# SanPen/CSparse3

Measured on AMD Instinct MI355X. Metric: numeric-LU + lsolve/usolve nnz/s on 50k power-grid Jacobian, higher is better.
Workload: dtype f64; 1 GPU; configs[2]: synthetic banded power-grid Jacobian 50000x50000, 501330 nnz, LU refactor + 1-RHS solve per step, one matrix per GPU; n=50000, nnz_a=501330, nnz_l=696852, nnz_u=696852, rhs=1, supernodes=5970, levels=12, max_front=469, ordering=amd(A+A')

## Files before the change

csparse3_amd/csrc/kernels.hip:

```cpp
#include <hip/hip_runtime.h>


#include <stdint.h>

#include <algorithm>
#include <cstdlib>

#include "cs3_device.hpp"
#include "cs3_devfn.hpp"

namespace cs3 {

hipError_t set_withhold_handover(int on)
{
    hipError_t e = hipMemcpyToSymbol(HIP_SYMBOL(g_withhold_handover), &on, sizeof(int));
    return e != hipSuccess ? e : set_withhold_handover_forest(on);
}

typedef double double4_t __attribute__((ext_vector_type(4)));

__device__ __forceinline__ double *il_lane_base(const IlView &il, long long m)
{
    return il.base + (m >> 6) * 64 * il.len + (m & 63);
}
// ... 2123 lines not shown
        us[j] = load_if(L, off, row < kb && jj < bw);
    }
    {
        constexpr int QW = BIG_KT / 4;
        BlockTriangle<KIND, false> ta;
        ta.load(L, r, kb, bw);
        double vi[QW];
#pragma unroll
        for (int u = 0; u < QW; ++u) {
            const int q = wv * QW + u;
            vi[u] = load_if(v0 + (long long) (q < nlive ? q : 0) * bv_size, kb + lane, lane < bw && q < nlive);
        }
        ta.template solve_multi<QW>(vi, bw);
#pragma unroll
        for (int u = 0; u < QW; ++u) y[wv * QW + u][lane] = (lane < bw) ? vi[u] : 0.0;
    }
    __syncthreads();
    if (blockIdx.x == 0 && tid < bw)
        for (int q = 0; q < nlive; ++q)
            X_all[(long long) b * x_stride + (long long) (d.c0 + kb + tid) * nrhs + rhs0 + q] = y[q][tid];
#pragma unroll
    for (int q = 0; q < BIG_KT; ++q) {
        double acc = 0.0;
#pragma unroll
        for (int j = 0; j < 16; ++j) acc += us[j] * y[q][wv * 16 + j];
        part[wv][q][lane] = acc;
    }
    __syncthreads();
    if (tid < 64 && row < kb)
        for (int q = 0; q < nlive; ++q) {
            double *vq = v0 + (long long) q * bv_size;
            vq[row] -= ((part[0][q][tid] + part[1][q][tid]) + part[2][q][tid]) + part[3][q][tid];
        }
}

template <int KIND>
__global__ void __launch_bounds__(256)
k_bwd_big_init(const SolveDesc *__restrict__ sd, int first, const int *__restrict__ st_idx,
               const double *__restrict__ pool_all, const double *__restrict__ X_all, double *__restrict__ bigv_all,
               int nrhs, long long pool_stride, long long x_stride, long long bv_size)
{
    extern __shared__ __attribute__((aligned(16))) double v2[];
    const SolveDesc d = sd[first + blockIdx.z];
    const int b = blockIdx.y / nrhs, rhs = blockIdx.y % nrhs;
    const int r = d.r, w = d.w, nb = r - w;
    const double *pool = pool_all + (long long) b * pool_stride;
    const double *X = X_all + (long long) b * x_stride;
    double *v = bigv_all + ((long long) b * nrhs + rhs) * bv_size + d.bv;
    const int *st = st_idx + d.st;
    const int tid = threadIdx.x;
    for (int j = tid; j < nb; j += 256) v2[j] = X[(long long) st[w + j] * nrhs + rhs];
    __syncthreads();
    const double *L = pool + d.lpan;
    const double *U = pool + d.upan;
    for (int i = blockIdx.x * 256 + tid; i < w; i += gridDim.x * 256) {
        double acc = 0.0;
        for (int j0 = 0; j0 < nb; j0 += 16) {
            double u[16];
#pragma unroll
            for (int j = 0; j < 16; ++j) {
                const int jj = j0 + j;
                const long long off = (KIND == CS3_LU) ? (long long) i * d.u_sk + (long long) jj * d.u_sj
                                                       : (long long) (w + jj) + (long long) i * r;
                u[j] = load_if((KIND == CS3_LU) ? U : L, off, jj < nb);
            }
#pragma unroll
            for (int j = 0; j < 16; ++j) acc += u[j] * v2[j0 + j < nb ? j0 + j : 0];
        }
        v[i] = X[(long long) (d.c0 + i) * nrhs + rhs] - acc;
    }
}

template <int KIND, int CW>
__global__ void __launch_bounds__(256)
k_bwd_big_step(const SolveDesc *__restrict__ sd, int first, int chunk_from_right,
               const double *__restrict__ pool_all, double *__restrict__ X_all, double *__restrict__ bigv_all,
               int nrhs, long long pool_stride, long long x_stride, long long bv_size)
{
    constexpr int SC = CW / 4;
    __shared__ double y[BIG_CW];
    __shared__ double cpl[64];
    __shared__ double part[4][64];
    const SolveDesc d = sd[first + blockIdx.z];
    const int r = d.r, w = d.w;
    const int nchunk = (w + CW - 1) / CW;
    const int c = nchunk - 1 - chunk_from_right;
    if (c < 0) return;
    const int kb = c * CW, bw = min(CW, w - kb);
    const int bwa = min(SOLVE_BW, bw), bwb = bw - bwa;
    const int nsl = (kb + 63) / 64;
    if ((int) blockIdx.x > 0 && (int) blockIdx.x >= nsl) return;
    const int b = blockIdx.y / nrhs, rhs = blockIdx.y % nrhs;
    const double *L = pool_all + (long long) b * pool_stride + d.lpan;
    double *v = bigv_all + ((long long) b * nrhs + rhs) * bv_size + d.bv;
    const int tid = threadIdx.x, lane = tid & 63, wv = tid >> 6;
    const int row = blockIdx.x * 64 + lane;
    double us[SC];
#pragma unroll
    for (int j = 0; j < SC; ++j) {
        const int jj = wv * SC + j;
        const long long off = (KIND == CS3_LU) ? (long long) row + (long long) (kb + jj) * r
                                               : (long long) (kb + jj) + (long long) row * r;
        us[j] = load_if(L, off, row < kb && jj < bw);
    }
    if (wv == 0) {
        if (bwb > 0) {
            BlockTriangle<KIND, false> tb;
            tb.load(L, r, kb + SOLVE_BW, bwb);
            const double vi = tb.solve(load_if(v, kb + SOLVE_BW + lane, lane < bwb), bwb);
            if (lane < bwb) y[SOLVE_BW + lane] = vi;
        }
        __syncthreads();
        __syncthreads();
    } else if (wv == 1) {
        BlockTriangle<KIND, false> ta;
        ta.load(L, r, kb, bwa);
        __syncthreads();
        __syncthreads();
        const double vi = ta.solve(cpl[lane], bwa);
        if (lane < bwa) y[lane] = vi;
    } else if (wv == 2) {
        double tm[SOLVE_BW];
#pragma unroll
        for (int j = 0; j < SOLVE_BW; ++j) {
            const long long i = kb + lane, k = kb + SOLVE_BW + j;
            const long long off = (KIND == CS3_LU) ? i + k * r : k + i * r;
            tm[j] = load_if(L, off, lane < bwa && j < bwb);
        }
        double vi = load_if(v, kb + lane, lane < bwa);
        __syncthreads();
#pragma unroll
        for (int j = 0; j < SOLVE_BW; ++j) vi -= tm[j] * ((j < bwb) ? y[SOLVE_BW + j] : 0.0);
        cpl[lane] = vi;
        __syncthreads();
    } else {
        __syncthreads();
        __syncthreads();
    }
    __syncthreads();
    if (blockIdx.x == 0 && tid < bw)
        X_all[(long long) b * x_stride + (long long) (d.c0 + kb + tid) * nrhs + rhs] = y[tid];
    double acc = 0.0;
#pragma unroll
    for (int j = 0; j < SC; ++j) {
        const int jj = wv * SC + j;
        acc += us[j] * y[jj < bw ? jj : 0];
    }
    part[wv][lane] = acc;
    __syncthreads();
    if (tid < 64 && row < kb)
        v[row] -= ((part[0][tid] + part[1][tid]) + part[2][tid]) + part[3][tid];
}

constexpr int IL_KB = 4;
constexpr int IL_T = 8;
constexpr int IL_TJ = 4;
constexpr int IL_NONE = INT32_MIN;
constexpr int IL_AV = 32;

template <int KIND, class Rule>
__global__ void __launch_bounds__(64)
k_front_il(const FrontDesc *__restrict__ fdesc, int first, const int *__restrict__ pairs,
           const double *__restrict__ ax_all, long long nnz_a, IlView il,
           const double *__restrict__ pool_pm_all, long long pm_stride, int batch, Rule rule, int *status)
{
    const double inv_tol = rule.inv_tol;
    const FrontDesc d = fdesc[first + blockIdx.x];
    const int lane = threadIdx.x;
    const long long m = (long long) blockIdx.y * 64 + lane;
    const bool live = m < batch;
    const long long mm = live ? m : (long long) blockIdx.y * 64;
    double *G = il.base + (long long) blockIdx.y * 64 * il.len + lane;
    const double *P = pool_pm_all + mm * pm_stride;
    const double *ax = ax_all + mm * nnz_a;
    const int r = d.r, w = d.w;
    double *F = G + d.lpan * 64;
#define EL(i, j) F[((long long) (i) + (long long) (j) * r) * 64]

    {
        const int np = d.a_count;
        const int *pr = pairs + 2 * d.a_begin;
        int cur = -1;
        double acc = 0.0;
        int ptg_n = pr[2 * (lane < min(64, np) ? lane : 0)], psr_n = pr[2 * (lane < min(64, np) ? lane : 0) + 1];
        for (int base = 0; base < np; base += 64) {
            const int have = min(64, np - base);
            const int ptg = ptg_n, psr = psr_n;
            if (base + 64 < np) {
                const int have_n = min(64, np - base - 64);
                const int e_n = base + 64 + (lane < have_n ? lane : 0);
                ptg_n = pr[2 * e_n]; psr_n = pr[2 * e_n + 1];
            }
            for (int c = 0; c < have; c += IL_AV) {
                double val[IL_AV];
#pragma unroll
                for (int u = 0; u < IL_AV; ++u) {
                    const int sr = bcast_lane_i(psr, (c + u) & 63);
                    const bool none = sr == IL_NONE;
                    const int sc = none ? 0 : sr;
                    const double *p = (sc >= 0) ? ((sc < il.len) ? (const double *) (G + (long long) sc * 64) : P + sc) : ax + ~sc;
                    const double v = *p;
                    val[u] = none ? 0.0 : v;
                }
#pragma unroll
                for (int u = 0; u < IL_AV; ++u) {
                    if (c + u >= have) break;
                    const int tg = bcast_lane_i(ptg, c + u);
                    if (tg != cur) {
                        if (cur >= 0) F[(long long) cur * 64] = acc;
                        cur = tg; acc = 0.0;
                    }
                    acc += (tg >= 0) ? val[u] : 0.0;
                }
            }
        }
        if (cur >= 0) F[(long long) cur * 64] = acc;
    }

    bool bad = false;
    int bad_col = 0, hits = 0;
    for (int k0 = 0; k0 < w; k0 += IL_KB) {
        const int kb = min(IL_KB, w - k0), ke = k0 + kb;
        double dd[IL_KB][IL_KB], rd[IL_KB];
#pragma unroll
        for (int jj = 0; jj < IL_KB; ++jj)
#pragma unroll
            for (int ii = 0; ii < IL_KB; ++ii) {
                const bool in = ii < kb && jj < kb && (KIND == CS3_LU || ii >= jj);
                const double v = EL(in ? k0 + ii : k0, in ? k0 + jj : k0);
                dd[jj][ii] = in ? v : ((ii == jj) ? 1.0 : 0.0);
            }
#pragma unroll
        for (int kk = 0; kk < IL_KB; ++kk) {
            double piv = dd[kk][kk];
            if constexpr (Rule::on) {
                if (kk < kb) {
                    const bool hit = perturb_pivot(rule, piv);
                    dd[kk][kk] = piv;
                    hits += (int) hit;
                }
            }
            double dg;
            pivot_scale<KIND>(piv, dg, rd[kk]);
            bool rej = (KIND == CS3_LU) ? (!(fabs(piv) > 0.0) || !(fabs(piv) < 1.0e300)) : !(piv > 0.0);
            if (KIND == CS3_CHOLESKY) dd[kk][kk] = (piv > 0.0) ? dg : -1.0;
#pragma unroll
            for (int ii = kk + 1; ii < IL_KB; ++ii) {
                dd[kk][ii] *= rd[kk];
                if (KIND == CS3_LU) rej = rej || (ii < kb && !(fabs(dd[kk][ii]) <= inv_tol));
            }
            if (rej && kk < kb) { bad_col = bad ? min(bad_col, k0 + kk) : k0 + kk; bad = true; }
#pragma unroll
            for (int jj = kk + 1; jj < IL_KB; ++jj)
#pragma unroll
                for (int ii = (KIND == CS3_LU ? kk + 1 : jj); ii < IL_KB; ++ii)
                    dd[jj][ii] -= dd[kk][ii] * ((KIND == CS3_LU) ? dd[jj][kk] : dd[kk][jj]);
        }
#pragma unroll
        for (int jj = 0; jj < IL_KB; ++jj)
#pragma unroll
            for (int ii = 0; ii < IL_KB; ++ii)
                if (ii < kb && jj < kb && (KIND == CS3_LU || ii >= jj)) EL(k0 + ii, k0 + jj) = dd[jj][ii];
        for (int i0 = ke; i0 < r; i0 += IL_T) {
            double t[IL_T][IL_KB];
#pragma unroll
            for (int a = 0; a < IL_T; ++a)
#pragma unroll
                for (int jj = 0; jj < IL_KB; ++jj) {
                    const bool in = i0 + a < r && jj < kb;
                    const double v = EL(in ? i0 + a : i0, in ? k0 + jj : k0);
                    t[a][jj] = in ? v : 0.0;
                }
#pragma unroll
            for (int a = 0; a < IL_T; ++a)
#pragma unroll
                for (int jj = 0; jj < IL_KB; ++jj) {
                    double x = t[a][jj];
#pragma unroll
                    for (int kk = 0; kk < jj; ++kk) x -= t[a][kk] * ((KIND == CS3_LU) ? dd[jj][kk] : dd[kk][jj]);
                    x *= rd[jj];
                    t[a][jj] = x;
                    if (KIND == CS3_LU && jj < kb && i0 + a < r && !(fabs(x) <= inv_tol)) { bad_col = bad ? min(bad_col, k0 + jj) : k0 + jj; bad = true; }
                }
#pragma unroll
            for (int a = 0; a < IL_T; ++a)
#pragma unroll
                for (int jj = 0; jj < IL_KB; ++jj)
                    if (i0 + a < r && jj < kb) EL(i0 + a, k0 + jj) = t[a][jj];
        }
        if (KIND == CS3_LU) {
            for (int j0 = ke; j0 < r; j0 += IL_T) {
                double u[IL_T][IL_KB];
#pragma unroll
                for (int b = 0; b < IL_T; ++b)
#pragma unroll
                    for (int kk = 0; kk < IL_KB; ++kk) {
                        const bool in = j0 + b < r && kk < kb;
                        const double v = EL(in ? k0 + kk : k0, in ? j0 + b : k0);
                        u[b][kk] = in ? v : 0.0;
                    }
#pragma unroll
                for (int b = 0; b < IL_T; ++b)
#pragma unroll
                    for (int kk = 1; kk < IL_KB; ++kk) {
                        double x = u[b][kk];
#pragma unroll
// ... 882 lines not shown
        break;
    }
    });
#undef CS3_FRONT_ARGS
    CS3_LAUNCH_CHECK();
    return hipSuccess;
}

__global__ void __launch_bounds__(256) k_poison_lds(int words)
{
    extern __shared__ __attribute__((aligned(16))) double pz[];
    for (int i = threadIdx.x; i < words; i += 256) pz[i] = __longlong_as_double(0x7ff8dead0000beefll);
    __syncthreads();
    if (pz[(threadIdx.x * 97) % words] == 0.0) pz[0] = 1.0;
}

hipError_t launch_poison_lds(hipStream_t st)
{
    const int bytes = 160 * 1024;
    hipError_t e = hipFuncSetAttribute((const void *) k_poison_lds, hipFuncAttributeMaxDynamicSharedMemorySize, bytes);
    if (e != hipSuccess) return e;
    hipLaunchKernelGGL(k_poison_lds, dim3(1024), dim3(256), bytes, st, bytes / 8);
    CS3_LAUNCH_CHECK();
    return hipSuccess;
}

hipError_t prepare_kernels()
{
    const int big = 160 * 1024;
    hipError_t e;
    using Plain = PivotRule<false>;
    using Perturbed = PivotRule<true>;
    const void *block_fns[] = {(const void *) k_front_block<CS3_LU, Plain, 16>, (const void *) k_front_block<CS3_LU, Perturbed, 16>,
                               (const void *) k_front_block<CS3_CHOLESKY, Plain, 16>,
                               (const void *) k_front_block<CS3_CHOLESKY, Plain, 16, 4>,
                               (const void *) k_front_wg<CS3_LU, Plain, WG_NB>, (const void *) k_front_wg<CS3_LU, Perturbed, WG_NB>,
                               (const void *) k_front_wg<CS3_CHOLESKY, Plain, WG_NB>};
    for (const void *f : block_fns) {
        e = hipFuncSetAttribute(f, hipFuncAttributeMaxDynamicSharedMemorySize, big);
        if (e != hipSuccess) return e;
    }
    const void *gemm_fns[] = {(const void *) k_gemm_fwd<CS3_LU>, (const void *) k_gemm_fwd<CS3_CHOLESKY>,
                              (const void *) k_gemm_bwd<CS3_LU>, (const void *) k_gemm_bwd<CS3_CHOLESKY>,
                              (const void *) k_gemm_bwd_init<CS3_LU>, (const void *) k_gemm_bwd_init<CS3_CHOLESKY>};
    for (const void *f : gemm_fns) {
        e = hipFuncSetAttribute(f, hipFuncAttributeMaxDynamicSharedMemorySize, big);
        if (e != hipSuccess) return e;
    }
    const void *solve_fns[] = {
        (const void *) k_fwd_blk<CS3_LU>, (const void *) k_fwd_blk<CS3_CHOLESKY>,
        (const void *) k_bwd_blk<CS3_LU>, (const void *) k_bwd_blk<CS3_CHOLESKY>,
        (const void *) k_bwd_big_init<CS3_LU>, (const void *) k_bwd_big_init<CS3_CHOLESKY>};
    for (const void *f : solve_fns) {
        e = hipFuncSetAttribute(f, hipFuncAttributeMaxDynamicSharedMemorySize, big);
        if (e != hipSuccess) return e;
    }
    return hipSuccess;
}

hipError_t ForkJoin::init()
{
    for (int i = 0; i < NSIDE; ++i) {
        hipError_t e = hipStreamCreateWithFlags(&side[i], hipStreamNonBlocking);
        if (e != hipSuccess) return e;
    }
    return hipStreamCreateWithFlags(&aux, hipStreamNonBlocking);
}

void ForkJoin::destroy()
{
    for (int i = 0; i < NSIDE; ++i) if (side[i]) { (void) hipStreamDestroy(side[i]); side[i] = nullptr; }
    if (aux) { (void) hipStreamDestroy(aux); aux = nullptr; }
    for (hipEvent_t e : events) (void) hipEventDestroy(e);
    events.clear();
    next = 0;
}

hipError_t ForkJoin::event(hipEvent_t *out)
{
    if (next == events.size()) {
        hipEvent_t e;
        hipError_t rc = hipEventCreateWithFlags(&e, hipEventDisableTiming);
        if (rc != hipSuccess) return rc;
        events.push_back(e);
    }
    *out = events[next++];
    return hipSuccess;
}

static size_t level_edge(const std::vector<LaunchGroup> &groups, size_t g, bool forward)
{
    const int level = groups[forward ? g : g - 1].level;
    if (forward) while (g < groups.size() && groups[g].level == level) ++g;
    else while (g > 0 && groups[g - 1].level == level) --g;
    return g;
}

template <class F>
static auto with_sweep_kind(int kind, bool trans, F &&f)
{
    if (kind == CS3_LU && trans) return f(std::integral_constant<int, CS3_LU_T>{});
    return with_kind(kind, f);
}

template <class Launch>
static hipError_t run_level(const std::vector<LaunchGroup> &groups, size_t g0, size_t g1, hipStream_t st,
                            ForkJoin &fj, bool parallel, Launch launch)
{
    const size_t ng = g1 - g0;
    if (ng <= 1) return ng ? launch(groups[g0], st) : hipSuccess;
    if (!parallel) {
        for (size_t i = g0; i < g1; ++i) { hipError_t e = launch(groups[i], st); if (e != hipSuccess) return e; }
        return hipSuccess;
    }
    hipEvent_t fork;
    hipError_t e = fj.event(&fork);
    if (e != hipSuccess) return e;
    if ((e = hipEventRecord(fork, st)) != hipSuccess) return e;
    if ((e = launch(groups[g1 - 1], st)) != hipSuccess) return e;
    for (size_t i = 0; i + 1 < ng; ++i) {
        hipStream_t s = fj.side[i % ForkJoin::NSIDE];
        if (i < (size_t) ForkJoin::NSIDE) { if ((e = hipStreamWaitEvent(s, fork, 0)) != hipSuccess) return e; }
        if ((e = launch(groups[g0 + i], s)) != hipSuccess) return e;
    }
    for (size_t i = 0; i < std::min(ng - 1, (size_t) ForkJoin::NSIDE); ++i) {
        hipEvent_t j;
        if ((e = fj.event(&j)) != hipSuccess) return e;
        if ((e = hipEventRecord(j, fj.side[i])) != hipSuccess) return e;
        if ((e = hipStreamWaitEvent(st, j, 0)) != hipSuccess) return e;
    }
    return hipSuccess;
}

static std::vector<LaunchGroup> factor_groups(const DeviceFactor &D, const std::vector<LaunchGroup> &groups);

hipError_t launch_factor_levels(const DeviceFactor &D, const SweepCall &call, const std::vector<LaunchGroup> &all_groups,
                                const PivotCtl &pc, hipStream_t st, ForkJoin &fj)
{
    const std::vector<LaunchGroup> groups = factor_groups(D, all_groups);
    fj.rewind();
    for (size_t g0 = 0; g0 < groups.size(); ) {
        const size_t g1 = level_edge(groups, g0, true);
        hipError_t e = run_level(groups, g0, g1, st, fj, true, [&](const LaunchGroup &g, hipStream_t s) {
            return with_kind(D.kind, [&](auto K) { return launch_front_group<K>(D, call, g, pc, s); });
        });
        if (e != hipSuccess) return e;
        g0 = g1;
    }
    return hipSuccess;
}

struct BigSweepPlan {
    bool wide, multi;
    int cw, nchunk, slices;
    unsigned by, by_multi;
};

static BigSweepPlan big_sweep_plan(const DeviceFactor &D, const LaunchGroup &g, int nrhs)
{
    BigSweepPlan pl;
    pl.by = (unsigned) (D.batch * nrhs);
    pl.wide = (long long) D.batch * nrhs < 8;
    pl.multi = nrhs >= BIG_KT;
    pl.by_multi = (unsigned) (D.batch * ((nrhs + BIG_KT - 1) / BIG_KT));
    pl.cw = pl.wide ? BIG_CW : SOLVE_BW;
    pl.nchunk = (g.max_w + pl.cw - 1) / pl.cw;
    pl.slices = std::max(1, (g.max_r + 63) / 64);
    return pl;
}

static hipError_t launch_fwd_big_pre(const DeviceFactor &D, const SweepCall &call, const LaunchGroup &g, double *X, int nrhs, hipStream_t st)
{
    const BigSweepPlan pl = big_sweep_plan(D, g, nrhs);
    hipLaunchKernelGGL(k_fwd_big_gather, dim3(1, pl.by, g.count), dim3(256), 0, st, call.sd, g.first, D.fasm_src,
                       D.fasm_tgt, D.flong_src, D.cv, X, D.bigv, nrhs, D.cv_size * (long long) nrhs, D.n * (long long) nrhs, D.bv_size);
    CS3_LAUNCH_CHECK();
    return hipSuccess;
}

template <int KIND>
static hipError_t launch_fwd_big_chunk(const DeviceFactor &D, const SweepCall &call, const LaunchGroup &g, double *X, int nrhs, int c,
                                       hipStream_t st)
{
    const BigSweepPlan pl = big_sweep_plan(D, g, nrhs);
    const long long xs = D.n * (long long) nrhs, cvs = D.cv_size * (long long) nrhs;
    if (pl.wide)
        hipLaunchKernelGGL((k_fwd_big_step<KIND, BIG_CW>), dim3(pl.slices, pl.by, g.count), dim3(256), 0, st, call.sd,
                           g.first, c * pl.cw, D.pool_pm, D.cv, X, D.bigv, nrhs, D.pm_stride, cvs, xs, D.bv_size);
    else if (pl.multi)
        hipLaunchKernelGGL((k_fwd_big_step_multi<KIND>), dim3(pl.slices, pl.by_multi, g.count), dim3(256), 0, st, call.sd,
                           g.first, c * pl.cw, D.pool_pm, D.cv, X, D.bigv, nrhs, D.pm_stride, cvs, xs, D.bv_size);
    else
        hipLaunchKernelGGL((k_fwd_big_step<KIND, SOLVE_BW>), dim3(pl.slices, pl.by, g.count), dim3(256), 0, st, call.sd,
                           g.first, c * pl.cw, D.pool_pm, D.cv, X, D.bigv, nrhs, D.pm_stride, cvs, xs, D.bv_size);
    CS3_LAUNCH_CHECK();
    return hipSuccess;
}

template <int KIND>
static hipError_t launch_bwd_big_pre(const DeviceFactor &D, const SweepCall &call, const LaunchGroup &g, double *X, int nrhs, hipStream_t st)
{
    const BigSweepPlan pl = big_sweep_plan(D, g, nrhs);
    const size_t lds = (size_t) std::max(1, g.max_r) * sizeof(double);
    hipLaunchKernelGGL((k_bwd_big_init<KIND>), dim3(2, pl.by, g.count), dim3(256), lds, st, call.sd, g.first,
                       D.st_idx, D.pool_pm, X, D.bigv, nrhs, D.pm_stride, D.n * (long long) nrhs, D.bv_size);
    CS3_LAUNCH_CHECK();
    return hipSuccess;
}

template <int KIND>
static hipError_t launch_bwd_big_chunk(const DeviceFactor &D, const SweepCall &call, const LaunchGroup &g, double *X, int nrhs, int c,
                                       hipStream_t st)
{
    const BigSweepPlan pl = big_sweep_plan(D, g, nrhs);
    const long long xs = D.n * (long long) nrhs;
    if (pl.wide)
        hipLaunchKernelGGL((k_bwd_big_step<KIND, BIG_CW>), dim3(pl.slices, pl.by, g.count), dim3(256), 0, st, call.sd,
                           g.first, c, D.pool_pm, X, D.bigv, nrhs, D.pm_stride, xs, D.bv_size);
    else if (pl.multi)
        hipLaunchKernelGGL((k_bwd_big_step_multi<KIND>), dim3(pl.slices, pl.by_multi, g.count), dim3(256), 0, st, call.sd,
                           g.first, c, D.pool_pm, X, D.bigv, nrhs, D.pm_stride, xs, D.bv_size);
    else
        hipLaunchKernelGGL((k_bwd_big_step<KIND, SOLVE_BW>), dim3(pl.slices, pl.by, g.count), dim3(256), 0, st, call.sd,
                           g.first, c, D.pool_pm, X, D.bigv, nrhs, D.pm_stride, xs, D.bv_size);
    CS3_LAUNCH_CHECK();
    return hipSuccess;
}


template <int KIND>
static hipError_t launch_inv_tasks(const DeviceFactor &D, int t0, int t1, hipStream_t st)
{
    if (t1 <= t0) return hipSuccess;
    hipLaunchKernelGGL((k_inv_diag<KIND>), dim3((unsigned) (t1 - t0), (unsigned) D.batch), dim3(256), 0, st, D.sdesc, D.inv_tasks, t0,
                       D.pool_pm, D.pm_stride, D.dinv, D.dinv_size);
    CS3_LAUNCH_CHECK();
    return hipSuccess;
}

static bool gemm_sweeps_on()
{
    static const bool on = !(getenv("CS3_NO_GEMM_SWEEPS") && getenv("CS3_NO_GEMM_SWEEPS")[0] == '1');
    return on;
}

bool permutation_can_fuse(const DeviceFactor &D, int nrhs)
{
    constexpr int min_rhs = 256;
    return gemm_sweeps_on() && nrhs >= std::max(min_rhs, RHS_LANES_MIN) && D.il_len == 0;
}

hipError_t launch_diag_inverses(const DeviceFactor &D, hipStream_t st)
{
    return with_kind(D.kind, [&](auto K) { return launch_inv_tasks<K>(D, 0, D.n_inv_tasks, st); });
}

template <int KIND>
static hipError_t launch_gemm_group(const DeviceFactor &D, const SweepCall &call, const LaunchGroup &g, double *X, int nrhs,
                                    bool forward, hipStream_t st)
{
    const long long xs = D.n * (long long) nrhs, cvs = D.cv_size * (long long) nrhs, gvs = D.gv_size * (long long) nrhs;
    const unsigned batch = (unsigned) D.batch, tiles = (unsigned) ((nrhs + GC - 1) / GC);
    int t0 = 0, t1 = 0;
    {
        const std::vector<int> &T = D.inv_tasks_host;
        const int nt = (int) (T.size() / 2);
        while (t0 < nt && T[2 * t0] < g.first) ++t0;
        t1 = t0;
        while (t1 < nt && T[2 * t1] < g.first + g.count) ++t1;
    }
    if (forward && call.inverses_in_sweep) {
        hipError_t ie = launch_inv_tasks<(KIND == CS3_LU_T) ? CS3_LU : KIND>(D, t0, t1, st);
        if (ie != hipSuccess) return ie;
    }
    const int nchunk = (g.max_w + GC - 1) / GC;
    const unsigned slices = (unsigned) std::max(1, (g.max_r + GC - 1) / GC);
    if (forward) {
        hipLaunchKernelGGL(k_gemm_gather, dim3((unsigned) ((g.max_r + 15) / 16), tiles, g.count * batch), dim3(256), 0, st, call.sd,
                           g.first, D.sl_src, D.cv, X, D.gv, nrhs, cvs, xs, gvs, call.xm, (int) batch);
        CS3_LAUNCH_CHECK();
        for (int c = 0; c < nchunk; ++c) {
            hipLaunchKernelGGL((k_gemm_fwd<KIND>), dim3(slices, tiles, g.count * batch), dim3(512), GEMM_LDS, st, call.sd, g.first, c,
                               D.pool_pm, D.dinv, D.cv, X, D.gv, nrhs, D.pm_stride, D.dinv_size, cvs, xs, gvs, (int) batch);
            CS3_LAUNCH_CHECK();
        }
    } else {
        hipLaunchKernelGGL((k_gemm_bwd_init<KIND>), dim3((unsigned) nchunk, tiles, g.count * batch), dim3(512), GEMM_LDS, st, call.sd,
                           g.first, D.st_idx, D.pool_pm, X, D.gv, nrhs, D.pm_stride, xs, gvs, (int) batch);
        CS3_LAUNCH_CHECK();
        for (int c = 0; c < nchunk; ++c) {
            hipLaunchKernelGGL((k_gemm_bwd<KIND>), dim3((unsigned) std::max(1, nchunk), tiles, g.count * batch), dim3(512), GEMM_LDS, st,
                               call.sd, g.first, c, D.pool_pm, D.dinv, X, D.gv, nrhs, D.pm_stride, D.dinv_size, xs, gvs, (int) batch, call.xm);
            CS3_LAUNCH_CHECK();
        }
    }
    return hipSuccess;
}

template <int KIND, int RMAX>
static void launch_rhs_sweep(const DeviceFactor &D, const SweepCall &call, int first, int count, double *X, int nrhs, bool forward, hipStream_t st)
{
    if (count <= 0) return;
    const long long xs = D.n * (long long) nrhs, cvs = D.cv_size * (long long) nrhs;
    dim3 grid((unsigned) count, (unsigned) D.batch, (unsigned) ((nrhs + 63) / 64));
    if (forward)
        hipLaunchKernelGGL((k_fwd_rhs<KIND, RMAX>), grid, dim3(64), 0, st, call.sd, first, D.sl_src, D.pool_pm, D.cv, X,
                           nrhs, D.pm_stride, cvs, xs, call.xm);
    else
        hipLaunchKernelGGL((k_bwd_rhs<KIND, RMAX>), grid, dim3(64), 0, st, call.sd, first, D.st_idx, D.pool_pm, X,
                           nrhs, D.pm_stride, xs, call.xm);
}

template <int KIND>
static hipError_t launch_solve_group(const DeviceFactor &D, const SweepCall &call, const LaunchGroup &g, double *X, int nrhs,
                                     bool forward, hipStream_t st)
{
    const long long xs = D.n * (long long) nrhs;
    const long long cvs = D.cv_size * (long long) nrhs;
    if (g.cls == SK_SUB) return (nrhs == 1 && KIND != CS3_LU_T) ? launch_sub_sweep(D, X, forward, st) : hipErrorInvalidValue;
    if (gemm_sweeps_on() && nrhs >= RHS_LANES_MIN && (g.cls == SK_WAVE || g.cls == SK_BLOCK || g.cls == SK_BIG))
        return launch_gemm_group<KIND>(D, call, g, X, nrhs, forward, st);
    if (g.cls == SK_IL) {
        const int n16 = g.n16;
        if (n16 > 0) {
            dim3 grid((unsigned) n16, (unsigned) D.ngroups);
            if (forward)
                hipLaunchKernelGGL((k_fwd_il<KIND, 16>), grid, dim3(64), 0, st, call.sd, g.first, D.rl_pairs,
                                   IlView{D.pool_il, D.il_len}, D.cv, X, nrhs, cvs, xs, (int) D.batch);
            else
                hipLaunchKernelGGL((k_bwd_il<KIND, 16>), grid, dim3(64), 0, st, call.sd, g.first, D.st_idx,
                                   IlView{D.pool_il, D.il_len}, X, nrhs, xs, (int) D.batch);
        }
        if (g.count > n16) {
            dim3 grid((unsigned) (g.count - n16), (unsigned) D.ngroups);
            if (forward)
                hipLaunchKernelGGL((k_fwd_il<KIND, IL_RMAX>), grid, dim3(64), 0, st, call.sd, g.first + n16, D.rl_pairs,
                                   IlView{D.pool_il, D.il_len}, D.cv, X, nrhs, cvs, xs, (int) D.batch);
            else
                hipLaunchKernelGGL((k_bwd_il<KIND, IL_RMAX>), grid, dim3(64), 0, st, call.sd, g.first + n16, D.st_idx,
                                   IlView{D.pool_il, D.il_len}, X, nrhs, xs, (int) D.batch);
        }
    } else if (g.cls == SK_SMALL && nrhs >= RHS_LANES_MIN) {
        if (g.max_r <= 16) launch_rhs_sweep<KIND, 16>(D, call, g.first, g.count, X, nrhs, forward, st);
        else if (g.max_r <= 24) launch_rhs_sweep<KIND, 24>(D, call, g.first, g.count, X, nrhs, forward, st);
        else if (g.max_r <= 32) launch_rhs_sweep<KIND, 32>(D, call, g.first, g.count, X, nrhs, forward, st);
        else return hipErrorInvalidValue;
    } else if (g.cls == SK_SMALL || g.cls == SK_WAVE) {
        if (nrhs == 1) {
            dim3 grid((unsigned) ((g.count + 3) / 4), (unsigned) D.batch, 1);
            if (forward)
                hipLaunchKernelGGL((k_fwd_wave<KIND, 1>), grid, dim3(256), 0, st, call.sd, g.first, g.count, D.fasm_src,
                                   D.fasm_tgt, D.flong_src, D.pool_pm, D.cv, X, nrhs, D.pm_stride, cvs, xs);
            else
                hipLaunchKernelGGL((k_bwd_wave<KIND, 1>), grid, dim3(256), 0, st, call.sd, g.first, g.count, D.st_idx,
                                   D.pool_pm, X, nrhs, D.pm_stride, xs);
        } else {
            constexpr int KT = 8;
            dim3 grid((unsigned) ((g.count + 3) / 4), (unsigned) D.batch, (unsigned) ((nrhs + KT - 1) / KT));
            if (forward)
                hipLaunchKernelGGL((k_fwd_wave<KIND, KT>), grid, dim3(256), 0, st, call.sd, g.first, g.count, D.fasm_src,
                                   D.fasm_tgt, D.flong_src, D.pool_pm, D.cv, X, nrhs, D.pm_stride, cvs, xs);
            else
                hipLaunchKernelGGL((k_bwd_wave<KIND, KT>), grid, dim3(256), 0, st, call.sd, g.first, g.count, D.st_idx,
                                   D.pool_pm, X, nrhs, D.pm_stride, xs);
        }
    } else if (g.cls == SK_BIG) {
        const BigSweepPlan pl = big_sweep_plan(D, g, nrhs);
        hipError_t e = forward ? launch_fwd_big_pre(D, call, g, X, nrhs, st) : launch_bwd_big_pre<KIND>(D, call, g, X, nrhs, st);
        for (int c = 0; e == hipSuccess && c < pl.nchunk; ++c)
            e = forward ? launch_fwd_big_chunk<KIND>(D, call, g, X, nrhs, c, st) : launch_bwd_big_chunk<KIND>(D, call, g, X, nrhs, c, st);
        return e;
    } else {
        dim3 grid((unsigned) g.count, (unsigned) D.batch, (unsigned) nrhs);
        const size_t lds = (size_t) (g.max_r + 1 + SOLVE_BW) * sizeof(double);
        if (forward)
            hipLaunchKernelGGL((k_fwd_blk<KIND>), grid, dim3(256), lds, st, call.sd, g.first, D.fasm_src,
                               D.fasm_tgt, D.flong_src, D.pool_pm, D.cv, X, nrhs, D.pm_stride, cvs, xs);
        else
            hipLaunchKernelGGL((k_bwd_blk<KIND>), grid, dim3(256), lds, st, call.sd, g.first, D.st_idx,
                               D.pool_pm, X, nrhs, D.pm_stride, xs);
    }
    CS3_LAUNCH_CHECK();
    return hipSuccess;
}

static int promote_max()
{
    return 16;
}

static void absorb_small_group(std::vector<LaunchGroup> &out, const LaunchGroup &g, int small_cls, int wg_cls)
{
    if (!out.empty() && out.back().level == g.level && out.back().cls == small_cls && g.cls == wg_cls &&
        out.back().count <= promote_max() && out.back().first + out.back().count == g.first) {
        LaunchGroup &m = out.back();
        m.cls = wg_cls; m.count += g.count;
        m.max_r = std::max(m.max_r, g.max_r); m.max_w = std::max(m.max_w, g.max_w);
        m.n16 = 0;
    } else {
        out.push_back(g);
    }
}

static std::vector<LaunchGroup> sweep_groups(const std::vector<LaunchGroup> &groups, int nrhs, long long batch)
{
    if (nrhs >= RHS_LANES_MIN) return groups;
    std::vector<LaunchGroup> merged, out;
    for (const LaunchGroup &g : groups) {
        if (!merged.empty() && merged.back().level == g.level && merged.back().cls == SK_SMALL && g.cls == SK_WAVE &&
            merged.back().first + merged.back().count == g.first) {
            LaunchGroup &m = merged.back();
            m.cls = SK_WAVE; m.count += g.count;
            m.max_r = std::max(m.max_r, g.max_r); m.max_w = std::max(m.max_w, g.max_w);
        } else {
            merged.push_back(g);
        }
    }
    if (batch != 1) return merged;
    for (const LaunchGroup &g : merged) absorb_small_group(out, g, SK_WAVE, SK_BLOCK);
    return out;
}

static std::vector<LaunchGroup> factor_groups(const DeviceFactor &D, const std::vector<LaunchGroup> &groups)
{
    if (D.batch != 1) return groups;
    std::vector<LaunchGroup> out;
    for (const LaunchGroup &g : groups) absorb_small_group(out, g, FC_R64, FC_LDS);
    return out;
}

hipError_t launch_solve_levels(const DeviceFactor &D, const SweepCall &call, double *X, int nrhs, bool forward, hipStream_t st, ForkJoin &fj)
{
    const std::vector<LaunchGroup> groups = sweep_groups(*call.groups, nrhs, D.batch);
    fj.rewind();
    const bool solve_parallel = nrhs >= 512;
    auto launch = [&](const LaunchGroup &g, hipStream_t s) {
        return with_sweep_kind(D.kind, call.trans, [&](auto K) { return launch_solve_group<K>(D, call, g, X, nrhs, forward, s); });
    };
    if (forward) {
        for (size_t g0 = 0; g0 < groups.size(); ) {
            const size_t g1 = level_edge(groups, g0, true);
            hipError_t e = run_level(groups, g0, g1, st, fj, solve_parallel, launch);
            if (e != hipSuccess) return e;
            g0 = g1;
        }
    } else {
        for (size_t g1 = groups.size(); g1 > 0; ) {
            const size_t g0 = level_edge(groups, g1, false);
            hipError_t e = run_level(groups, g0, g1, st, fj, solve_parallel, launch);
            if (e != hipSuccess) return e;
            g1 = g0;
        }
    }
    return hipSuccess;
}

static int factor_group_cost(const LaunchGroup &g)
{
    return (g.cls == FC_BIG) ? 4 * ((g.max_w + BIG_NB - 1) / BIG_NB + 2) : 2;
}
static int sweep_group_cost(const LaunchGroup &g)
{
    return (g.cls == SK_BIG) ? 2 + (g.max_w + BIG_CW - 1) / BIG_CW : 1;
}

hipError_t launch_factor_with_forward(const DeviceFactor &D, const SweepCall &call, const std::vector<LaunchGroup> &all_fgroups,
                                      const PivotCtl &pc, double *X, int nrhs, hipStream_t st, ForkJoin &fj)
{
    hipError_t e;
    if (!D.sub_forest.empty() && call.sd != D.sdesc1) {
        if ((e = launch_factor_levels(D, call, all_fgroups, pc, st, fj)) != hipSuccess) return e;
        return launch_solve_levels(D, call, X, nrhs, true, st, fj);
    }
    const std::vector<LaunchGroup> fgroups = factor_groups(D, all_fgroups);
    const std::vector<LaunchGroup> sgroups = sweep_groups(*call.groups, nrhs, D.batch);
    fj.rewind();
    const int nlevels = fgroups.empty() ? 0 : fgroups.back().level + 1;
    std::vector<long long> tail(nlevels + 1, 0), head(nlevels + 1, 0);
    for (const LaunchGroup &g : fgroups) tail[g.level] += factor_group_cost(g);
    for (int l = nlevels - 1; l >= 0; --l) tail[l] += tail[l + 1];
    for (const LaunchGroup &g : sgroups) head[g.level + 1] += (g.cls == SK_SUB && call.fwd_in_factor) ? 0 : sweep_group_cost(g);
    for (int l = 0; l < nlevels; ++l) head[l + 1] += head[l];
    int fork_level = -1;
    static const bool overlap = !(getenv("CS3_NO_OVERLAP") && getenv("CS3_NO_OVERLAP")[0] == '1');
    for (int l = 0; overlap && l + 1 < nlevels; ++l)
        if (tail[l + 1] >= head[l + 1]) fork_level = l;

    auto sweep = [&](int lo, int hi, hipStream_t s) -> hipError_t {
        for (const LaunchGroup &g : sgroups) {
            if (g.level < lo || g.level > hi) continue;
            if (g.cls == SK_SUB && call.fwd_in_factor) continue;
            hipError_t se = with_sweep_kind(D.kind, call.trans,
                                            [&](auto K) { return launch_solve_group<K>(D, call, g, X, nrhs, true, s); });
            if (se != hipSuccess) return se;
        }
        return hipSuccess;
    };
    if (overlap && D.batch >= 16 && nlevels >= 2) {
        hipEvent_t pending = nullptr;
        int pending_level = -1;
        auto flush = [&]() -> hipError_t {
            if (!pending) return hipSuccess;
            hipError_t fe;
            if ((fe = hipStreamWaitEvent(fj.aux, pending, 0)) != hipSuccess) return fe;
            fe = sweep(pending_level, pending_level, fj.aux);
            pending = nullptr;
            return fe;
        };
        for (size_t f0 = 0; f0 < fgroups.size(); ) {
            const int level = fgroups[f0].level;
            const size_t f1 = level_edge(fgroups, f0, true);
            e = run_level(fgroups, f0, f1, st, fj, true, [&](const LaunchGroup &g, hipStream_t s2) {
                return with_kind(D.kind, [&](auto K) { return launch_front_group<K>(D, call, g, pc, s2); });
            });
            if (e != hipSuccess) return e;
            if ((e = flush()) != hipSuccess) return e;
            if ((e = fj.event(&pending)) != hipSuccess) return e;
            if ((e = hipEventRecord(pending, st)) != hipSuccess) return e;
            pending_level = level;
            f0 = f1;
        }
// ... 149 lines not shown
```

Before: 4.470 billion nnz/s.

## Add 512-thread four-block chunk kernels for wide big-front triangular sweeps

For big supernodes wider than BIG_CW with a single RHS, the forward and backward sweeps now use new 512-thread kernels. Each processes a chunk four SOLVE_BW blocks wide, with wavefronts pipelining the diagonal-block triangular solves against the off-diagonal coupling tiles. This cuts the number of sequential chunk launches per front, and the row-slice height drops to 32 so more blocks run in parallel. When the group is a single square front, the backward init kernel is skipped and the first chunks read their inputs directly through an xmode flag. The cost is many extra barriers, more complex synchronisation, and more register pressure.

```diff
diff --git a/csparse3_amd/csrc/kernels.hip b/csparse3_amd/csrc/kernels.hip
--- a/csparse3_amd/csrc/kernels.hip
+++ b/csparse3_amd/csrc/kernels.hip
@@ -2299,6 +2299,229 @@
         v[row] -= ((part[0][tid] + part[1][tid]) + part[2][tid]) + part[3][tid];
 }
 
+constexpr int BIG_CW4 = 4 * SOLVE_BW;
+constexpr int BIG_SR4 = 32;
+
+__device__ __forceinline__ double load_at(const double *__restrict__ base, unsigned byte_off)
+{
+    return *reinterpret_cast<const double *>(reinterpret_cast<const char *>(base) + byte_off);
+}
+
+template <int KIND, bool FORWARD, bool TRI = false>
+__device__ __forceinline__ void load_chunk_tile(double (&tm)[SOLVE_BW], const double *__restrict__ L, int r, int kb, int rb,
+                                                int cb, int bw)
+{
+    constexpr bool by_column = FORWARD ? (KIND != CS3_LU_T) : (KIND == CS3_LU);
+    const int lane = threadIdx.x & 63;
+    const int i = kb + SOLVE_BW * rb + lane, k0 = kb + SOLVE_BW * cb;
+    const bool row_in = SOLVE_BW * rb + lane < bw;
+    const int ncol = min(SOLVE_BW, max(0, bw - SOLVE_BW * cb));
+    if constexpr (by_column) {
+        const unsigned off = row_in ? 8u * (unsigned) i : 0u;
+#pragma unroll
+        for (int j = 0; j < SOLVE_BW; ++j) {
+            const double x = load_at(L + (j < ncol ? (long long) (k0 + j) * r : 0), off);
+            tm[j] = (row_in && j < ncol && (!TRI || (FORWARD ? lane > j : lane < j))) ? x : 0.0;
+        }
+    } else {
+        const double *row = L + (row_in ? (long long) i * r + k0 : 0);
+#pragma unroll
+        for (int j = 0; j < SOLVE_BW; ++j) {
+            const double x = row[j < ncol ? j : 0];
+            tm[j] = (row_in && j < ncol && (!TRI || (FORWARD ? lane > j : lane < j))) ? x : 0.0;
+        }
+    }
+}
+
+template <int KIND, bool FORWARD>
+__device__ __forceinline__ void load_chunk_triangle(BlockTriangle<KIND, FORWARD> &tri, const double *__restrict__ L, int r, int kb,
+                                                    int b, int bw)
+{
+    const int lane = threadIdx.x & 63;
+    tri.rdg = tri.DIAG ? recip_diag(L, kb + SOLVE_BW * b + lane, r, SOLVE_BW * b + lane < bw) : 1.0;
+    load_chunk_tile<KIND, FORWARD, true>(tri.t, L, r, kb, b, b, bw);
+    if (tri.DIAG) {
+#pragma unroll
+        for (int j = 0; j < SOLVE_BW; ++j) tri.t[j] *= tri.rdg;
+    }
+}
+
+__device__ __forceinline__ double chunk_tile_dot(const double (&tm)[SOLVE_BW], const double *__restrict__ yb, double acc)
+{
+#pragma unroll
+    for (int j = 0; j < SOLVE_BW; ++j) acc -= tm[j] * yb[j];
+    return acc;
+}
+
+template <int KIND, bool FORWARD, class Rhs>
+__device__ __forceinline__ void solve_chunk4(const double *__restrict__ L, int r, int kb, int bw, Rhs rhs, double *y,
+                                             double (*cpl)[SOLVE_BW], double (*far)[SOLVE_BW])
+{
+    const int lane = threadIdx.x & 63, wv = threadIdx.x >> 6;
+    auto blk = [](int s) { return FORWARD ? s : 3 - s; };
+    auto wid = [&](int b) { return min(SOLVE_BW, max(0, bw - SOLVE_BW * b)); };
+    auto row = [&](int b) { return kb + SOLVE_BW * b + lane; };
+    if (wv < 4) {
+        const int b = blk(wv), bwb = wid(b);
+        BlockTriangle<KIND, FORWARD> tri;
+        load_chunk_triangle(tri, L, r, kb, b, bw);
+        if (wv == 0) {
+            double vi = rhs(row(b), lane < bwb);
+            if (bwb > 0) vi = tri.solve(vi, bwb);
+            y[SOLVE_BW * b + lane] = (lane < bwb) ? vi : 0.0;
+            __syncthreads();
+            double tm[SOLVE_BW];
+            load_chunk_tile<KIND, FORWARD>(tm, L, r, kb, blk(3), b, bw);
+            __syncthreads();
+            __syncthreads();
+            far[1][lane] = -chunk_tile_dot(tm, y + SOLVE_BW * b, 0.0);
+            __syncthreads();
+            __syncthreads();
+            __syncthreads();
+            __syncthreads();
+        } else {
+            for (int s = 0; s < 2 * wv; ++s) __syncthreads();
+            double vi = cpl[wv][lane];
+            if (bwb > 0) vi = tri.solve(vi, bwb);
+            y[SOLVE_BW * b + lane] = (lane < bwb) ? vi : 0.0;
+            for (int s = 2 * wv; s < 7; ++s) __syncthreads();
+        }
+    } else if (wv < 7) {
+        const int s = wv - 3, b = blk(s), a = blk(s - 1);
+        double tm[SOLVE_BW];
+        load_chunk_tile<KIND, FORWARD>(tm, L, r, kb, b, a, bw);
+        double vi = rhs(row(b), lane < wid(b));
+        for (int t = 0; t < 2 * s - 1; ++t) __syncthreads();
+        if (s == 2) vi -= far[0][lane];
+        if (s == 3) vi = (vi - far[1][lane]) - far[2][lane];
+        cpl[s][lane] = chunk_tile_dot(tm, y + SOLVE_BW * a, vi);
+        for (int t = 2 * s - 1; t < 7; ++t) __syncthreads();
+    } else {
+        double tm[SOLVE_BW];
+        load_chunk_tile<KIND, FORWARD>(tm, L, r, kb, blk(2), blk(0), bw);
+        __syncthreads();
+        far[0][lane] = -chunk_tile_dot(tm, y + SOLVE_BW * blk(0), 0.0);
+        double tn[SOLVE_BW];
+        load_chunk_tile<KIND, FORWARD>(tn, L, r, kb, blk(3), blk(1), bw);
+        __syncthreads();
+        __syncthreads();
+        far[2][lane] = -chunk_tile_dot(tn, y + SOLVE_BW * blk(1), 0.0);
+        __syncthreads();
+        __syncthreads();
+        __syncthreads();
+        __syncthreads();
+    }
+}
+
+template <int KIND>
+__global__ void __launch_bounds__(512)
+k_fwd_big_step4(const SolveDesc *__restrict__ sd, int first, int kb,
+                const double *__restrict__ pool_all, double *__restrict__ cv_all, double *__restrict__ X_all,
+                double *__restrict__ bigv_all, int nrhs, long long pool_stride, long long cv_stride,
+                long long x_stride, long long bv_size)
+{
+    constexpr int SC = BIG_CW4 / 16;
+    __shared__ double y[BIG_CW4];
+    __shared__ double cpl[4][SOLVE_BW];
+    __shared__ double far[3][SOLVE_BW];
+    __shared__ double part[16][BIG_SR4];
+    const SolveDesc d = sd[first + blockIdx.z];
+    const int r = d.r, w = d.w;
+    if (kb >= w) return;
+    const int bw = min(BIG_CW4, w - kb), ke = kb + bw;
+    const int nsl = (r - ke + BIG_SR4 - 1) / BIG_SR4;
+    if ((int) blockIdx.x > 0 && (int) blockIdx.x >= nsl) return;
+    const int b = blockIdx.y / nrhs, rhs = blockIdx.y % nrhs;
+    const double *L = pool_all + (long long) b * pool_stride + d.lpan;
+    double *v = bigv_all + ((long long) b * nrhs + rhs) * bv_size + d.bv;
+    const int tid = threadIdx.x;
+    const int cg = tid / BIG_SR4, row = ke + blockIdx.x * BIG_SR4 + tid % BIG_SR4;
+    double ls[SC];
+#pragma unroll
+    for (int j = 0; j < SC; ++j) {
+        const int jj = cg * SC + j;
+        if constexpr (KIND == CS3_LU_T) ls[j] = u_entry(L, pool_all + (long long) b * pool_stride + d.upan, d, kb + jj, row, row < r && jj < bw);
+        else ls[j] = (row < r && jj < bw) ? load_at(L + (jj < bw ? (long long) (kb + jj) * r : 0), row < r ? 8u * (unsigned) row : 0u) : 0.0;
+    }
+    const double old = load_if(v, row, cg == 0 && row < r);
+    solve_chunk4<KIND, true>(L, r, kb, bw, [&](int i, bool p) { return load_if(v, i, p); }, y, cpl, far);
+    if (blockIdx.x == 0 && tid < bw)
+        X_all[(long long) b * x_stride + (long long) (d.c0 + kb + tid) * nrhs + rhs] = y[tid];
+    double acc = 0.0;
+#pragma unroll
+    for (int j = 0; j < SC; ++j) acc += ls[j] * y[cg * SC + j];
+    part[cg][tid % BIG_SR4] = acc;
+    __syncthreads();
+    if (cg == 0 && row < r) {
+        double sum = part[0][tid];
+#pragma unroll
+        for (int q = 1; q < 16; ++q) sum += part[q][tid];
+        const double nv = old - sum;
+        v[row] = nv;
+        if (ke >= w && row >= w && d.parent >= 0)
+            cv_all[(long long) b * cv_stride + (d.cv + row - w) * nrhs + rhs] = nv;
+    }
+}
+
+template <int KIND>
+__global__ void __launch_bounds__(512)
+k_bwd_big_step4(const SolveDesc *__restrict__ sd, int first, int chunk_from_right, int xmode,
+                const double *__restrict__ pool_all, double *__restrict__ X_all, double *__restrict__ bigv_all,
+                int nrhs, long long pool_stride, long long x_stride, long long bv_size)
+{
+    constexpr int SC = BIG_CW4 / 16;
+    __shared__ double y[BIG_CW4];
+    __shared__ double cpl[4][SOLVE_BW];
+    __shared__ double far[3][SOLVE_BW];
+    __shared__ double part[16][BIG_SR4];
+    const SolveDesc d = sd[first + blockIdx.z];
+    const int r = d.r, w = d.w;
+    const int nchunk = (w + BIG_CW4 - 1) / BIG_CW4;
+    const int c = nchunk - 1 - chunk_from_right;
+    if (c < 0) return;
+    const int kb = c * BIG_CW4, bw = min(BIG_CW4, w - kb), ke = kb + bw;
+    const int nsl = (kb + BIG_SR4 - 1) / BIG_SR4;
+    if ((int) blockIdx.x > 0 && (int) blockIdx.x >= nsl) return;
+    const int b = blockIdx.y / nrhs, rhs = blockIdx.y % nrhs;
+    const double *L = pool_all + (long long) b * pool_stride + d.lpan;
+    double *v = bigv_all + ((long long) b * nrhs + rhs) * bv_size + d.bv;
+    double *X = X_all + (long long) b * x_stride;
+    const int tid = threadIdx.x;
+    const int cg = tid / BIG_SR4, row = blockIdx.x * BIG_SR4 + tid % BIG_SR4;
+    double us[SC];
+#pragma unroll
+    for (int j = 0; j < SC; ++j) {
+        const int jj = cg * SC + j;
+        if constexpr (KIND == CS3_LU)
+            us[j] = (row < kb && jj < bw) ? load_at(L + (jj < bw ? (long long) (kb + jj) * r : 0), row < kb ? 8u * (unsigned) row : 0u) : 0.0;
+        else
+            us[j] = load_if(L, (long long) (kb + jj) + (long long) row * r, row < kb && jj < bw);
+    }
+    auto before = [&](int i, bool p) {
+        return (xmode == 1) ? load_if(X, (long long) (d.c0 + i) * nrhs + rhs, p) : load_if(v, i, p);
+    };
+    const double old = before(row, cg == 0 && row < kb);
+    const bool parked = xmode == 2 && blockIdx.x == 0 && tid < min(BIG_CW4, w - ke);
+    const double home = load_if(v, ke + tid, parked);
+    solve_chunk4<KIND, false>(L, r, kb, bw, before, y, cpl, far);
+    if (parked) X[(long long) (d.c0 + ke + tid) * nrhs + rhs] = home;
+    if (blockIdx.x == 0 && tid < bw) {
+        if (xmode == 1 && nsl > 0) v[kb + tid] = y[tid];
+        else X[(long long) (d.c0 + kb + tid) * nrhs + rhs] = y[tid];
+    }
+    double acc = 0.0;
+#pragma unroll
+    for (int j = 0; j < SC; ++j) acc += us[j] * y[cg * SC + j];
+    part[cg][tid % BIG_SR4] = acc;
+    __syncthreads();
+    if (cg == 0 && row < kb) {
+        double sum = part[0][tid];
+#pragma unroll
+        for (int q = 1; q < 16; ++q) sum += part[q][tid];
+        v[row] = old - sum;
+    }
+}
+
 constexpr int IL_KB = 4;
 constexpr int IL_T = 8;
 constexpr int IL_TJ = 4;
@@ -3487,6 +3710,7 @@
 
 struct BigSweepPlan {
     bool wide, multi;
+    bool no_init;
     int cw, nchunk, slices;
     unsigned by, by_multi;
 };
@@ -3498,9 +3722,11 @@
     pl.wide = (long long) D.batch * nrhs < 8;
     pl.multi = nrhs >= BIG_KT;
     pl.by_multi = (unsigned) (D.batch * ((nrhs + BIG_KT - 1) / BIG_KT));
-    pl.cw = pl.wide ? BIG_CW : SOLVE_BW;
+    pl.cw = pl.wide ? (g.max_w > BIG_CW ? BIG_CW4 : BIG_CW) : SOLVE_BW;
+    pl.no_init = pl.cw == BIG_CW4 && g.count == 1 && g.max_r == g.max_w;
     pl.nchunk = (g.max_w + pl.cw - 1) / pl.cw;
-    pl.slices = std::max(1, (g.max_r + 63) / 64);
+    const int sr = (pl.cw == BIG_CW4) ? BIG_SR4 : 64;
+    pl.slices = std::max(1, (g.max_r + sr - 1) / sr);
     return pl;
 }
 
@@ -3519,7 +3745,10 @@
 {
     const BigSweepPlan pl = big_sweep_plan(D, g, nrhs);
     const long long xs = D.n * (long long) nrhs, cvs = D.cv_size * (long long) nrhs;
-    if (pl.wide)
+    if (pl.cw == BIG_CW4)
+        hipLaunchKernelGGL((k_fwd_big_step4<KIND>), dim3(pl.slices, pl.by, g.count), dim3(512), 0, st, call.sd,
+                           g.first, c * pl.cw, D.pool_pm, D.cv, X, D.bigv, nrhs, D.pm_stride, cvs, xs, D.bv_size);
+    else if (pl.wide)
         hipLaunchKernelGGL((k_fwd_big_step<KIND, BIG_CW>), dim3(pl.slices, pl.by, g.count), dim3(256), 0, st, call.sd,
                            g.first, c * pl.cw, D.pool_pm, D.cv, X, D.bigv, nrhs, D.pm_stride, cvs, xs, D.bv_size);
     else if (pl.multi)
@@ -3549,7 +3778,10 @@
 {
     const BigSweepPlan pl = big_sweep_plan(D, g, nrhs);
     const long long xs = D.n * (long long) nrhs;
-    if (pl.wide)
+    if (pl.cw == BIG_CW4)
+        hipLaunchKernelGGL((k_bwd_big_step4<KIND>), dim3(pl.slices, pl.by, g.count), dim3(512), 0, st, call.sd,
+                           g.first, c, (pl.no_init && c < 2) ? c + 1 : 0, D.pool_pm, X, D.bigv, nrhs, D.pm_stride, xs, D.bv_size);
+    else if (pl.wide)
         hipLaunchKernelGGL((k_bwd_big_step<KIND, BIG_CW>), dim3(pl.slices, pl.by, g.count), dim3(256), 0, st, call.sd,
                            g.first, c, D.pool_pm, X, D.bigv, nrhs, D.pm_stride, xs, D.bv_size);
     else if (pl.multi)
@@ -3701,7 +3933,8 @@
         }
     } else if (g.cls == SK_BIG) {
         const BigSweepPlan pl = big_sweep_plan(D, g, nrhs);
-        hipError_t e = forward ? launch_fwd_big_pre(D, call, g, X, nrhs, st) : launch_bwd_big_pre<KIND>(D, call, g, X, nrhs, st);
+        hipError_t e = forward ? launch_fwd_big_pre(D, call, g, X, nrhs, st)
+                               : pl.no_init ? hipSuccess : launch_bwd_big_pre<KIND>(D, call, g, X, nrhs, st);
         for (int c = 0; e == hipSuccess && c < pl.nchunk; ++c)
             e = forward ? launch_fwd_big_chunk<KIND>(D, call, g, X, nrhs, c, st) : launch_bwd_big_chunk<KIND>(D, call, g, X, nrhs, c, st);
         return e;
```

Measured after the change: 4.644 billion nnz/s (median of 6 runs). 1.04x the previous value.
